# tomneda/DABstar

Measured on NVIDIA B200. Metric: Mode I DAB frames/s decoded (IQ->Viterbi), higher is better.
Workload: dtype f32

## Files before the change

dabstar_b200/csrc/ofdm_kernels.cu:

```cuda
#include "fft2048.cuh"
#include "kernels.h"
#include "devcache.h"

#include <algorithm>
#include <cstdlib>
#include <type_traits>

namespace dab
{
namespace
{
template <int FMT> struct Raw;
template <> struct Raw<FMT_U8> { typedef unsigned short type; typedef unsigned reg; };
template <> struct Raw<FMT_I16> { typedef short2 type; typedef short2 reg; };
template <> struct Raw<FMT_CF32> { typedef float2 type; typedef float2 reg; };

__device__ __forceinline__ float2 to_cf(unsigned v)
{
  const float2 m = make_float2(__uint_as_float(__byte_perm(v, 0x4B000000u, 0x7540)), __uint_as_float(__byte_perm(v, 0x4B000000u, 0x7541)));
  const float2 f = __fadd2_rn(m, make_float2(-8388608.0f, -8388608.0f));
  return __ffma2_rn(f, make_float2(1.0f / 128.0f, 1.0f / 128.0f), make_float2(-127.38f / 128.0f, -127.38f / 128.0f));
}
__device__ __forceinline__ float2 to_cf(short2 v) { return __fmul2_rn(make_float2((float)v.x, (float)v.y), make_float2(1.0f / 32768.0f, 1.0f / 32768.0f)); }
__device__ __forceinline__ float2 to_cf(float2 v) { return v; }
// ... 645 lines not shown
  fft2048_to_smem(v, tw, smem, tid);
  for (int i = tid; i < T_U; i += FFT_THREADS) ref_arg_conj[i] = smem[fft_nat(i)];
}

struct CpInt
{
  int p1, p2, s1, s2;
};
__device__ __forceinline__ unsigned dp4a_uu(unsigned a, unsigned b, unsigned c)
{
  unsigned d;
  asm("dp4a.u32.u32 %0, %1, %2, %3;" : "=r"(d) : "r"(a), "r"(b), "r"(c));
  return d;
}
__device__ __forceinline__ int dp4a_us(unsigned a, unsigned b_signed, int c)
{
  int d;
  asm("dp4a.u32.s32 %0, %1, %2, %3;" : "=r"(d) : "r"(a), "r"(b_signed), "r"(c));
  return d;
}
__device__ __forceinline__ void cp_int_add(CpInt & t, unsigned aw, unsigned bw)
{
  t.p1 = (int)dp4a_uu(aw, bw, (unsigned)t.p1);
  const unsigned bs = __byte_perm(bw, 0u, 0x2301);
  t.p2 = (int)dp4a_uu(aw & 0xff00ff00u, bs, (unsigned)t.p2);
  t.p2 -= (int)dp4a_uu(aw & 0x00ff00ffu, bs, 0u);
  t.s1 = (int)dp4a_uu(aw, 0x01010101u, dp4a_uu(bw, 0x01010101u, (unsigned)t.s1));
  t.s2 = dp4a_us(aw, 0x01ff01ffu, dp4a_us(bw, 0xff01ff01u, t.s2));
}
__device__ __forceinline__ int warp_sum_int(int v)
{
#pragma unroll
  for (int o = 16; o > 0; o >>= 1) v += __shfl_xor_sync(0xffffffffu, v, o);
  return v;
}
__device__ __forceinline__ float2 cp_int_finish(const CpInt * red, int n_syms)
{
  long long p1 = 0, p2 = 0, s1 = 0, s2 = 0;
  for (int w = 0; w < 8; w++) { p1 += red[w].p1; p2 += red[w].p2; s1 += red[w].s1; s2 += red[w].s2; }
  const double c = 127.38, n = (double)n_syms * (double)T_G;
  return make_float2((float)(((double)p1 - c * (double)s1 + 2.0 * n * c * c) * (1.0 / 16384.0)), (float)(((double)p2 - c * (double)s2) * (1.0 / 16384.0)));
}

template <int FMT>
__global__ void __launch_bounds__(256) k_cp_corr(const FrameDesc * __restrict__ frames, int n_frames, const RecInput * __restrict__ recs, float2 * __restrict__ cp)
{
  __shared__ float2 red[8];
  __shared__ CpInt redi[8];
  for (int fi = blockIdx.x; fi < n_frames; fi += gridDim.x)
  {
    const FrameDesc fd = frames[fi];
    const RecInput rin = recs[fd.rec];
    const long long base = fd.sym0 + T_U;
    float2 acc = make_float2(0.0f, 0.0f);
    CpInt ti = { 0, 0, 0, 0 };
    typedef typename Raw<FMT>::type T;
    const int lane = threadIdx.x & 31;
    for (int sym = threadIdx.x >> 5; sym < fd.n_syms; sym += 8)
    {
      const T * pp = reinterpret_cast<const T *>(rin.iq) + base + (long long)sym * T_S + lane;
      typename Raw<FMT>::reg ra[16], rb[16];
#pragma unroll
      for (int k = 0; k < 16; k++)
      {
        if (lane + 32 * k < T_G) { ra[k] = pp[32 * k + T_U]; rb[k] = pp[32 * k]; }
        else { ra[k] = typename Raw<FMT>::reg(); rb[k] = typename Raw<FMT>::reg(); }
      }
#pragma unroll
      for (int k = 0; k < 16; k++)
      {
        if (lane + 32 * k < T_G)
        {
          if constexpr (FMT == FMT_U8) cp_int_add(ti, ra[k], rb[k]);
          else
          {
            const float2 a = to_cf(ra[k]), b = to_cf(rb[k]);
            acc.x += a.x * b.x + a.y * b.y;
            acc.y += a.y * b.x - a.x * b.y;
          }
        }
      }
    }
    if constexpr (FMT == FMT_U8)
    {
      ti.p1 = warp_sum_int(ti.p1); ti.p2 = warp_sum_int(ti.p2); ti.s1 = warp_sum_int(ti.s1); ti.s2 = warp_sum_int(ti.s2);
      if ((threadIdx.x & 31) == 0) redi[threadIdx.x >> 5] = ti;
      __syncthreads();
      if (threadIdx.x == 0) cp[fi] = cp_int_finish(redi, fd.n_syms);
    }
    else
    {
      acc.x = warp_sum(acc.x);
      acc.y = warp_sum(acc.y);
      if ((threadIdx.x & 31) == 0) red[threadIdx.x >> 5] = acc;
      __syncthreads();
      if (threadIdx.x == 0)
      {
        float2 s = red[0];
        for (int w = 1; w < 8; w++) { s.x += red[w].x; s.y += red[w].y; }
        cp[fi] = s;
      }
    }
    __syncthreads();
  }
}

constexpr int CPB_STAGES = 4;
constexpr int CPB_COPY = 1024;
constexpr int CPB_SMEM = 8 * CPB_STAGES * 2 * CPB_COPY;

__global__ void __launch_bounds__(256) k_cp_corr_bulk(const FrameDesc * __restrict__ frames, int n_frames, const RecInput * __restrict__ recs, float2 * __restrict__ cp)
{
  extern __shared__ __align__(128) unsigned char cpb_ring[];
  __shared__ unsigned long long cpb_bar[8 * CPB_STAGES];
  __shared__ CpInt red[8];
  const int lane = threadIdx.x & 31, warp = threadIdx.x >> 5;
  unsigned char * ring = cpb_ring + warp * (CPB_STAGES * 2 * CPB_COPY);
  const unsigned ring_s = smem_addr_u32(ring), bar_s = smem_addr_u32(cpb_bar + warp * CPB_STAGES);
  if (lane == 0)
  {
#pragma unroll
    for (int b = 0; b < CPB_STAGES; b++) mbar_init(bar_s + 8u * (unsigned)b, 1);
    asm volatile("fence.mbarrier_init.release.cluster;" ::: "memory");
    asm volatile("fence.proxy.async.shared::cta;" ::: "memory");
  }
  __syncthreads();

  struct Cursor
  {
    int fi, sym, n_syms;
    long long base, n;
    const unsigned char * iq;
  };
  auto enter = [&](Cursor & c) {
    while (c.fi < n_frames)
    {
      const FrameDesc & fd = frames[c.fi];
      c.n_syms = fd.n_syms;
      if (warp < c.n_syms)
      {
        const RecInput rin = recs[fd.rec];
        c.base = fd.sym0 + T_U;
        c.n = rin.n;
        c.iq = static_cast<const unsigned char *>(rin.iq);
        c.sym = warp;
        return;
      }
      c.fi += (int)gridDim.x;
    }
  };
  auto advance = [&](Cursor & c) {
    c.sym += 8;
    if (c.sym >= c.n_syms) { c.fi += (int)gridDim.x; enter(c); }
  };
  auto first_sample = [](const Cursor & c) { return c.base + (long long)c.sym * T_S; };
  auto by_copy = [&](const Cursor & c) { const long long s0 = first_sample(c); return s0 >= 8 && s0 + T_U + T_G + 8 <= c.n; };
  auto issue = [&](const Cursor & c, int b) {
    if (c.fi < n_frames && by_copy(c) && lane == 0)
    {
      const unsigned long long a = (unsigned long long)(c.iq + 2 * first_sample(c)) & ~15ull;
      const unsigned dst = ring_s + (unsigned)(b * 2 * CPB_COPY), bar = bar_s + 8u * (unsigned)b;
      mbar_expect_tx(bar, 2u * CPB_COPY);
      bulk_g2s(dst, reinterpret_cast<const void *>(a), CPB_COPY, bar);
      bulk_g2s(dst + CPB_COPY, reinterpret_cast<const void *>(a + 2ull * T_U), CPB_COPY, bar);
    }
  };

  Cursor ahead;
  ahead.fi = (int)blockIdx.x;
  ahead.sym = 0; ahead.n_syms = 0; ahead.base = 0; ahead.n = 0; ahead.iq = nullptr;
  enter(ahead);
  Cursor cur = ahead;
#pragma unroll 1
  for (int b = 0; b < CPB_STAGES && ahead.fi < n_frames; b++) { issue(ahead, b); advance(ahead); }
  int stage = 0;
  unsigned phase_bits = 0;

  for (int fi = blockIdx.x; fi < n_frames; fi += gridDim.x)
  {
    CpInt ti = { 0, 0, 0, 0 };
    const int n_syms = frames[fi].n_syms;
    while (cur.fi == fi)
    {
      if (by_copy(cur))
      {
        mbar_wait(bar_s + 8u * (unsigned)stage, (phase_bits >> stage) & 1u);
        phase_bits ^= 1u << stage;
        const int off = (int)((unsigned long long)(cur.iq + 2 * first_sample(cur)) & 15ull);
        const uint4 * sp = reinterpret_cast<const uint4 *>(ring + stage * 2 * CPB_COPY) + lane;
        uint4 va[2], vb[2];
#pragma unroll
        for (int it = 0; it < 2; it++) { vb[it] = sp[32 * it]; va[it] = sp[32 * it + CPB_COPY / 16]; }
        if (lane == 0)
        {
          unsigned * w = reinterpret_cast<unsigned *>(&va[0]);
          unsigned * u = reinterpret_cast<unsigned *>(&vb[0]);
#pragma unroll
          for (int j = 0; j < 4; j++)
          {
            const int drop = min(max(off - 4 * j, 0), 4);
            const unsigned m = drop >= 4 ? 0u : 0xffffffffu << (8 * drop);
            w[j] &= m;
            u[j] &= m;
          }
        }
        if (lane == 31)
        {
          unsigned * w = reinterpret_cast<unsigned *>(&va[1]);
          unsigned * u = reinterpret_cast<unsigned *>(&vb[1]);
#pragma unroll
          for (int j = 0; j < 4; j++)
          {
            const int keep = min(max(off - 4 * j, 0), 4);
            const unsigned m = keep >= 4 ? 0xffffffffu : ~(0xffffffffu << (8 * keep));
            w[j] &= m;
            u[j] &= m;
          }
        }
#pragma unroll
        for (int it = 0; it < 2; it++)
        {
          cp_int_add(ti, va[it].x, vb[it].x);
          cp_int_add(ti, va[it].y, vb[it].y);
          cp_int_add(ti, va[it].z, vb[it].z);
          cp_int_add(ti, va[it].w, vb[it].w);
        }
      }
      else
      {
        const unsigned short * pp = reinterpret_cast<const unsigned short *>(cur.iq) + first_sample(cur) + lane;
        unsigned ra[16], rb[16];
#pragma unroll
        for (int k = 0; k < 16; k++)
        {
          if (lane + 32 * k < T_G) { ra[k] = pp[32 * k + T_U]; rb[k] = pp[32 * k]; }
          else { ra[k] = 0; rb[k] = 0; }
        }
#pragma unroll
        for (int k = 0; k < 16; k++) cp_int_add(ti, ra[k], rb[k]);
      }
      __syncwarp();
      asm volatile("fence.proxy.async.shared::cta;" ::: "memory");
      issue(ahead, stage);
      if (ahead.fi < n_frames) advance(ahead);
      advance(cur);
      stage = stage + 1 == CPB_STAGES ? 0 : stage + 1;
    }
    ti.p1 = warp_sum_int(ti.p1); ti.p2 = warp_sum_int(ti.p2); ti.s1 = warp_sum_int(ti.s1); ti.s2 = warp_sum_int(ti.s2);
    if (lane == 0) red[warp] = ti;
    __syncthreads();
    if (threadIdx.x == 0) cp[fi] = cp_int_finish(red, n_syms);
    __syncthreads();
  }
}

constexpr int DM3_RING = 64;
constexpr int DM3_ROW4 = K_CARR / 2;

__device__ __forceinline__ float rcp_ftz(float a) { float r; asm("rcp.approx.ftz.f32 %0, %1;" : "=f"(r) : "f"(a)); return r; }
__device__ __forceinline__ float rsqrt_ftz(float a) { float r; asm("rsqrt.approx.ftz.f32 %0, %1;" : "=f"(r) : "f"(a)); return r; }
__device__ __forceinline__ float sqrt_ftz(float a) { float r; asm("sqrt.approx.ftz.f32 %0, %1;" : "=f"(r) : "f"(a)); return r; }

__device__ __forceinline__ unsigned long long ld_volatile_global_b64(const unsigned long long * p)
{
  unsigned long long v;
  asm volatile("ld.relaxed.gpu.global.b64 %0, [%1];" : "=l"(v) : "l"(p) : "memory");
  return v;
}
__device__ __forceinline__ void st_volatile_global_b64(unsigned long long * p, unsigned long long v)
{
  asm volatile("st.relaxed.gpu.global.b64 [%0], %1;" ::"l"(p), "l"(v) : "memory");
}

__device__ __forceinline__ float2 f2(float a) { return make_float2(a, a); }
__device__ __forceinline__ float2 neg2(float2 a) { return make_float2(-a.x, -a.y); }
__device__ __forceinline__ float2 add2(float2 a, float2 b) { return __fadd2_rn(a, b); }
__device__ __forceinline__ float2 mul2(float2 a, float2 b) { return __fmul2_rn(a, b); }
__device__ __forceinline__ float2 fma2(float2 a, float2 b, float2 c) { return __ffma2_rn(a, b, c); }

struct CarrierPair
{
  float2 integ, stddev, mean_pow, mean_sigma, null_pow;
};

__device__ __forceinline__ float2 folded_phase2(float2 re, float2 im)
{
  const float ax0 = fabsf(re.x), ay0 = fabsf(im.x), ax1 = fabsf(re.y), ay1 = fabsf(im.y);
  const float2 mn = make_float2(fminf(ax0, ay0), fminf(ax1, ay1));
  const float2 t = mul2(mn, make_float2(rcp_ftz(fmaxf(ax0, ay0)), rcp_ftz(fmaxf(ax1, ay1))));
  const float2 z = mul2(t, t);
  float2 p = f2(0.00681177107617259f);
  p = fma2(p, z, f2(-0.033604156225919724f));
  p = fma2(p, z, f2(0.07962360233068466f));
  p = fma2(p, z, f2(-0.13233338296413422f));
  p = fma2(p, z, f2(0.19807815551757812f));
  p = fma2(p, z, f2(-0.3331736922264099f));
  p = fma2(p, z, f2(0.9999961256980896f));
  const float2 a = mul2(p, t);
  const bool m0 = (ay0 > ax0) != ((__float_as_int(re.x) ^ __float_as_int(im.x)) < 0);
  const bool m1 = (ay1 > ax1) != ((__float_as_int(re.y) ^ __float_as_int(im.y)) < 0);
  return make_float2(m0 ? PI_2_F - a.x : a.x, m1 ? PI_2_F - a.y : a.y);
}

template <int SOFT>
__device__ __forceinline__ void dm4_pair(CarrierPair & st, float2 xr, float2 xi, float2 rr, float2 ri, float2 ref_abs, float2 ref_inv, float2 cterm,
                                         float2 & o_re, float2 & o_im, float2 & r_abs, float2 & pow_acc)
{
  constexpr float ALPHA = 0.005f;
  const float2 re = mul2(fma2(xi, ri, mul2(xr, rr)), ref_inv);
  const float2 im = mul2(fma2(neg2(xr), ri, mul2(xi, rr)), ref_inv);
  const float2 t = add2(cterm, st.integ), a2 = mul2(t, t);
  const float2 rx = fma2(a2, fma2(a2, f2(3.679168224334716796875e-2f), f2(-0.495580852031707763671875f)), f2(0.9994032382965087890625f));
  const float2 ry = mul2(neg2(t), fma2(a2, f2(-0.16034401953220367431640625f), f2(0.99903142452239990234375f)));
  const float2 zr = fma2(neg2(im), ry, mul2(re, rx));
  const float2 zi = fma2(im, rx, mul2(re, ry));
  const float2 dv = add2(folded_phase2(zr, zi), f2(-PI_4_F));
  const float2 in = fma2(dv, f2(0.2f * ALPHA), st.integ);
  st.integ = make_float2(fminf(fmaxf(in.x, -20.0f * RAD_PER_DEG_F), 20.0f * RAD_PER_DEG_F), fminf(fmaxf(in.y, -20.0f * RAD_PER_DEG_F), 20.0f * RAD_PER_DEG_F));
  st.stddev = fma2(fma2(dv, dv, neg2(st.stddev)), f2(ALPHA), st.stddev);
  const float2 pw = fma2(zr, zr, mul2(zi, zi));
  st.mean_pow = fma2(add2(pw, neg2(st.mean_pow)), f2(ALPHA), st.mean_pow);
  pow_acc = fma2(pow_acc, f2(POW_ALL_DECAY), pw);
  const float2 lvl = make_float2(sqrt_ftz(st.mean_pow.x), sqrt_ftz(st.mean_pow.y));
  const float2 dr = fma2(lvl, f2(-0.70710678118654752440f), make_float2(fabsf(zr.x), fabsf(zr.y)));
  const float2 di = fma2(lvl, f2(-0.70710678118654752440f), make_float2(fabsf(zi.x), fabsf(zi.y)));
  st.mean_sigma = fma2(add2(fma2(dr, dr, mul2(di, di)), neg2(st.mean_sigma)), f2(ALPHA), st.mean_sigma);
  float2 sig = add2(st.mean_pow, neg2(st.null_pow));
  if (sig.x <= 0.0f) sig.x = 0.1f;
  if (sig.y <= 0.0f) sig.y = 0.1f;
  const float2 inv_z = make_float2(rsqrt_ftz(pw.x), rsqrt_ftz(pw.y));
  float2 w1;
  if (SOFT == 2) w1 = ref_abs;
  else
  {
    const float2 den = mul2(fma2(sig, f2(0.7f), st.null_pow), st.mean_sigma);
    const float2 g = mul2(sig, make_float2(rcp_ftz(den.x), rcp_ftz(den.y)));
    if (SOFT == 1) w1 = mul2(ref_abs, g);
    else
    {
      const float2 q = mul2(ref_abs, inv_z);
      w1 = mul2(mul2(make_float2(sqrt_ftz(q.x), sqrt_ftz(q.y)), lvl), g);
    }
  }
  r_abs = mul2(mul2(pw, inv_z), w1);
  o_re = mul2(zr, w1);
  o_im = mul2(zi, w1);
}

__device__ __forceinline__ void dm4_fix_saturated(int & a, int & b, int & c, int & e)
{
  a = a == 0x7fffffff ? 0 : a; b = b == 0x7fffffff ? 0 : b; c = c == 0x7fffffff ? 0 : c; e = e == 0x7fffffff ? 0 : e;
}

constexpr int DM5_T = 128;
constexpr int DM5_SLICES = K_CARR / 4 / DM5_T;
constexpr int DM5_WARPS = K_CARR / 128;
constexpr int DM5_PF = 8;

__device__ __forceinline__ float dm5_total(const unsigned long long * slot, unsigned long long w, unsigned tag, int lane)
{
  while (__any_sync(0xffffffffu, lane < DM5_WARPS && (unsigned)(w >> 32) != tag)) w = ld_volatile_global_b64(slot + (lane < DM5_WARPS ? lane : 0));
  float v = lane < DM5_WARPS ? __uint_as_float((unsigned)w) : 0.0f;
#pragma unroll
  for (int o = 16; o > 0; o >>= 1) v += __shfl_xor_sync(0xffffffffu, v, o);
  return v;
}

template <int SOFT, int LAG, bool QUAL>
__global__ void __launch_bounds__(DM5_T, 4) k_demap5(const DemapWork * __restrict__ work, const FrameDesc * __restrict__ frames,
                                                      const uint8_t * __restrict__ null_is_tii, const float2 * __restrict__ X,
                                                      const int16_t * __restrict__ rel_of_k, OfdmStateDev * __restrict__ states,
                                                      int16_t * __restrict__ soft, unsigned long long * __restrict__ ring, unsigned * __restrict__ ticket,
                                                      FrameQualSnap * __restrict__ qsnap)
{
  constexpr int STASH = LAG + 1;
  constexpr int T = DM5_T;
  static_assert((STASH & (STASH - 1)) == 0, "stash depth must be a power of two");
  static_assert(DM3_RING > 2 * LAG + 2, "a ring slot must not be overwritten while a slower warp may still read it");
  extern __shared__ float4 dm5_smem[];
  __shared__ unsigned s_ticket;
  if (threadIdx.x == 0) s_ticket = atomicAdd(ticket, 1u);
  __syncthreads();
  float4 * stash = dm5_smem;
  float4 * rowbuf = dm5_smem + STASH * T * 2;
  int * orow_ring = reinterpret_cast<int *>(rowbuf + DM5_PF * T * 2) + (threadIdx.x >> 5);
  const int w = (int)s_ticket / DM5_SLICES, slice = (int)s_ticket - w * DM5_SLICES;
  const DemapWork wk = work[w];
  const int tid = threadIdx.x, lane = tid & 31;
  const int t_rec = slice * T + tid;
  const int gw = t_rec >> 5;
  const int k0 = 4 * t_rec;
  unsigned long long * my_ring = ring + (size_t)w * DM3_RING * DM5_WARPS;

  const OfdmStateDev & sd = states[wk.state_in];
  CarrierPair sa, sb;
  float2 pow_a = f2(0.f), pow_b = f2(0.f);
  if (wk.reset) sa = sb = CarrierPair{ f2(0.f), f2(0.f), f2(0.f), f2(0.f), f2(0.f) };
  else
  {
    const float4 v0 = *reinterpret_cast<const float4 *>(sd.integ + k0), v1 = *reinterpret_cast<const float4 *>(sd.stddev + k0),
                 v2 = *reinterpret_cast<const float4 *>(sd.mean_pow + k0), v3 = *reinterpret_cast<const float4 *>(sd.mean_sigma + k0),
                 v4 = *reinterpret_cast<const float4 *>(sd.null_pow + k0), v5 = *reinterpret_cast<const float4 *>(sd.pow_acc + k0);
    sa = CarrierPair{ make_float2(v0.x, v0.y), make_float2(v1.x, v1.y), make_float2(v2.x, v2.y), make_float2(v3.x, v3.y), make_float2(v4.x, v4.y) };
    sb = CarrierPair{ make_float2(v0.z, v0.w), make_float2(v1.z, v1.w), make_float2(v2.z, v2.w), make_float2(v3.z, v3.w), make_float2(v4.z, v4.w) };
    pow_a = make_float2(v5.x, v5.y);
    pow_b = make_float2(v5.z, v5.w);
  }
  const float mean_value0 = sd.mean_value;
  const float pow_carry0 = wk.reset ? 1.0f : sd.pow_carry;
  const float2 gka = make_float2((float)(K_CARR / 2 - rel_of_k[k0]) / (float)(K_CARR / 2), (float)(K_CARR / 2 - rel_of_k[k0 + 1]) / (float)(K_CARR / 2));
  const float2 gkb = make_float2((float)(K_CARR / 2 - rel_of_k[k0 + 2]) / (float)(K_CARR / 2), (float)(K_CARR / 2 - rel_of_k[k0 + 3]) / (float)(K_CARR / 2));
  constexpr float W2 = SOFT == 0 ? -100.0f : -140.0f;

  const int total_rows = wk.n_frames * X_ROWS;
  const float4 * rows = reinterpret_cast<const float4 *>(X + (size_t)(total_rows > 0 ? frames[wk.desc_first].xslot : 0) * X_ROWS * K_CARR) + 2 * t_rec;
  const unsigned rowbuf_addr = smem_addr_u32(rowbuf + 2 * tid);
#pragma unroll
  for (int i = 0; i < DM5_PF; i++)
  {
    if (i < total_rows)
    {
      cp_async16(rowbuf_addr + (unsigned)(i * T) * 32u, rows + (size_t)i * DM3_ROW4);
      cp_async16(rowbuf_addr + (unsigned)(i * T) * 32u + 16u, rows + (size_t)i * DM3_ROW4 + 1);
    }
    cp_async_commit();
  }

  float2 rra = f2(0.f), ria = f2(0.f), ref_abs_a = f2(0.f), ref_inv_a = f2(0.f);
  float2 rrb = f2(0.f), rib = f2(0.f), ref_abs_b = f2(0.f), ref_inv_b = f2(0.f);
  int g = 0;
  int q = 0;
  unsigned long long pre = 0;

  auto emit = [&](int d, int o_row, float total) {
    if (o_row < 0) return;
    const float w2 = d == 0 ? rcp_ftz(mean_value0) * W2 : rcp_ftz(total) * (W2 * (float)K_CARR);
    const float4 ra = stash[((d & (STASH - 1)) * T + tid) * 2], rb = stash[((d & (STASH - 1)) * T + tid) * 2 + 1];
    const float2 are = mul2(make_float2(ra.x, ra.y), f2(w2)), aim = mul2(make_float2(ra.z, ra.w), f2(w2));
    const float2 bre = mul2(make_float2(rb.x, rb.y), f2(w2)), bim = mul2(make_float2(rb.z, rb.w), f2(w2));
    int a0 = __float2int_rz(are.x), a1 = __float2int_rz(are.y), a2 = __float2int_rz(aim.x), a3 = __float2int_rz(aim.y);
    int b0 = __float2int_rz(bre.x), b1 = __float2int_rz(bre.y), b2 = __float2int_rz(bim.x), b3 = __float2int_rz(bim.y);
    if (max(max(max(a0, a1), max(a2, a3)), max(max(b0, b1), max(b2, b3))) == 0x7fffffff) { dm4_fix_saturated(a0, a1, a2, a3); dm4_fix_saturated(b0, b1, b2, b3); }
    int16_t * o = soft + (size_t)o_row * SYM_BITS;
    reinterpret_cast<uint2 *>(o)[t_rec] = make_uint2(__byte_perm((unsigned)a0, (unsigned)a1, 0x5410), __byte_perm((unsigned)b0, (unsigned)b1, 0x5410));
    reinterpret_cast<uint2 *>(o + K_CARR)[t_rec] = make_uint2(__byte_perm((unsigned)a2, (unsigned)a3, 0x5410), __byte_perm((unsigned)b2, (unsigned)b3, 0x5410));
  };
  auto wsum = [](float v) {
#pragma unroll
    for (int o = 16; o > 0; o >>= 1) v += __shfl_xor_sync(0xffffffffu, v, o);
    return v;
  };
  float4 cur_a, cur_b;
  auto next_row = [&]() {
    cp_async_wait<DM5_PF - 1>();
    const unsigned slot = (unsigned)((q & (DM5_PF - 1)) * T);
    cur_a = rowbuf[(slot + tid) * 2];
    cur_b = rowbuf[(slot + tid) * 2 + 1];
    if (q + DM5_PF < total_rows)
    {
      cp_async16(rowbuf_addr + slot * 32u, rows + (size_t)(q + DM5_PF) * DM3_ROW4);
      cp_async16(rowbuf_addr + slot * 32u + 16u, rows + (size_t)(q + DM5_PF) * DM3_ROW4 + 1);
    }
    cp_async_commit();
    q++;
  };
  auto set_reference = [&]() {
    rra = make_float2(cur_a.x, cur_a.y); ria = make_float2(cur_a.z, cur_a.w);
    rrb = make_float2(cur_b.x, cur_b.y); rib = make_float2(cur_b.z, cur_b.w);
    const float2 pa = fma2(rra, rra, mul2(ria, ria)), pb = fma2(rrb, rrb, mul2(rib, rib));
    ref_inv_a = make_float2(rsqrt_ftz(pa.x), rsqrt_ftz(pa.y));
    ref_inv_b = make_float2(rsqrt_ftz(pb.x), rsqrt_ftz(pb.y));
    ref_abs_a = mul2(pa, ref_inv_a);
    ref_abs_b = mul2(pb, ref_inv_b);
  };
  float part_prev = 0.0f;
  const bool upper = (lane & 16) != 0;
  int q_wait_g = -1, q_wait = 0;
  auto q_mean_value = [&](int d, float total) {
    if (QUAL && d == q_wait_g)
    {
      if (t_rec == 0) qsnap[q_wait].mean_value = total / (float)K_CARR;
      q_wait_g = -1;
    }
  };

  for (int fi = 0; fi < wk.n_frames; fi++)
  {
    const FrameDesc fd = frames[wk.desc_first + fi];
    const float cfac = fd.clock_err / 1024.0f * PI_F;
    const float2 cterm_a = mul2(f2(cfac), gka), cterm_b = mul2(f2(cfac), gkb);
    const int n_syms = fd.n_syms;
    const int out_row0 = fi < wk.warmup ? -(1 << 30) : fd.slot * 75;
    const bool tii = null_is_tii != nullptr && null_is_tii[wk.desc_first + fi];
    next_row();
    set_reference();
    for (int sym = 1; sym <= 75; sym++)
    {
      next_row();
      if (sym > n_syms) continue;
      const int d = g - LAG;
      const float b_in = lane < DM5_WARPS ? __uint_as_float((unsigned)pre) : 0.0f;
      const bool tags_ok = __all_sync(0xffffffffu, lane >= DM5_WARPS || (unsigned)(pre >> 32) == (unsigned)d);
      const unsigned long long pre_used = pre;
      if (d >= 0 && lane < DM5_WARPS) pre = ld_volatile_global_b64(my_ring + (size_t)(d & (DM3_RING - 1)) * DM5_WARPS + lane);
      float v = (upper ? b_in : part_prev) + __shfl_xor_sync(0xffffffffu, upper ? part_prev : b_in, 16);
#pragma unroll
      for (int o = 8; o > 0; o >>= 1) v += __shfl_xor_sync(0xffffffffu, v, o);
      const float tot_fast = __shfl_sync(0xffffffffu, v, 16);
      float2 a_re, a_im, a_abs, b_re, b_im, b_abs;
      dm4_pair<SOFT>(sa, make_float2(cur_a.x, cur_a.y), make_float2(cur_a.z, cur_a.w), rra, ria, ref_abs_a, ref_inv_a, cterm_a, a_re, a_im, a_abs, pow_a);
      dm4_pair<SOFT>(sb, make_float2(cur_b.x, cur_b.y), make_float2(cur_b.z, cur_b.w), rrb, rib, ref_abs_b, ref_inv_b, cterm_b, b_re, b_im, b_abs, pow_b);
      part_prev = (a_abs.x + a_abs.y) + (b_abs.x + b_abs.y);
      stash[((g & (STASH - 1)) * T + tid) * 2] = make_float4(a_re.x, a_re.y, a_im.x, a_im.y);
      stash[((g & (STASH - 1)) * T + tid) * 2 + 1] = make_float4(b_re.x, b_re.y, b_im.x, b_im.y);
      if (lane == 0) orow_ring[(g & (STASH - 1)) * (T >> 5)] = out_row0 + (sym - 1);
      __syncwarp();
      if (lane == 0 && g > 0)
        st_volatile_global_b64(my_ring + (size_t)((g - 1) & (DM3_RING - 1)) * DM5_WARPS + gw,
                               ((unsigned long long)(unsigned)g << 32) | (unsigned long long)__float_as_uint(v));
      if (d >= 0)
      {
        float tot = tot_fast;
        if (d > 0 && !tags_ok) tot = dm5_total(my_ring + (size_t)((d - 1) & (DM3_RING - 1)) * DM5_WARPS, pre_used, (unsigned)d, lane);
        emit(d, orow_ring[(d & (STASH - 1)) * (T >> 5)], tot);
        q_mean_value(d, tot);
      }
      g++;
      set_reference();
    }
    next_row();
    if (n_syms == 75 && !tii)
    {
      constexpr float MIN_POW = (1.0f / 32767.0f) * (1.0f / 32767.0f);
      const float2 xra = make_float2(cur_a.x, cur_a.y), xia = make_float2(cur_a.z, cur_a.w), xrb = make_float2(cur_b.x, cur_b.y), xib = make_float2(cur_b.z, cur_b.w);
      const float2 pa = add2(fma2(xra, xra, mul2(xia, xia)), f2(MIN_POW)), pb = add2(fma2(xrb, xrb, mul2(xib, xib)), f2(MIN_POW));
      sa.null_pow = fma2(add2(pa, neg2(sa.null_pow)), f2(0.05f), sa.null_pow);
      sb.null_pow = fma2(add2(pb, neg2(sb.null_pow)), f2(0.05f), sb.null_pow);
    }
    if (QUAL && out_row0 >= 0 && n_syms == 75)
    {
      FrameQualSnap & qs = qsnap[wk.desc_first + fi];
      *reinterpret_cast<float4 *>(qs.stddev + k0) = make_float4(sa.stddev.x, sa.stddev.y, sb.stddev.x, sb.stddev.y);
      *reinterpret_cast<float4 *>(qs.null_pow + k0) = make_float4(sa.null_pow.x, sa.null_pow.y, sb.null_pow.x, sb.null_pow.y);
      *reinterpret_cast<float4 *>(qs.pow_acc + k0) = make_float4(pow_a.x, pow_a.y, pow_b.x, pow_b.y);
      if (t_rec == 0) qs.pow_carry = pow_carry0 * powf(POW_ALL_DECAY, (float)g);
      q_wait_g = g;
      q_wait = wk.desc_first + fi;
    }
  }
  cp_async_wait<0>();
  if (g > 0)
  {
    const float part = wsum(part_prev);
    if (lane == 0)
      st_volatile_global_b64(my_ring + (size_t)((g - 1) & (DM3_RING - 1)) * DM5_WARPS + gw,
                             ((unsigned long long)(unsigned)g << 32) | (unsigned long long)__float_as_uint(part));
  }
#pragma unroll
  for (int i = LAG - 1; i >= 0; i--)
  {
    const int d = g - 1 - i;
    if (d < 0) continue;
    float tot = 0.0f;
    if (d >= 1)
    {
      const unsigned long long * slot = my_ring + (size_t)((d - 1) & (DM3_RING - 1)) * DM5_WARPS;
      unsigned long long word = 0;
      if (lane < DM5_WARPS) word = ld_volatile_global_b64(slot + lane);
      tot = dm5_total(slot, word, (unsigned)d, lane);
    }
    emit(d, orow_ring[(d & (STASH - 1)) * (T >> 5)], tot);
    q_mean_value(d, tot);
  }
  if (!QUAL && wk.state_out < 0) return;
  float tot_last = mean_value0 * (float)K_CARR;
  if (gw == 0 && g > 0)
  {
    unsigned long long word = 0;
    const unsigned long long * slot = my_ring + (size_t)((g - 1) & (DM3_RING - 1)) * DM5_WARPS;
    if (lane < DM5_WARPS) word = ld_volatile_global_b64(slot + lane);
    tot_last = dm5_total(slot, word, (unsigned)g, lane);
  }
  if (QUAL)
  {
    q_mean_value(g, tot_last);
    if (wk.state_out < 0) return;
  }
  OfdmStateDev & so = states[wk.state_out];
  *reinterpret_cast<float4 *>(so.integ + k0) = make_float4(sa.integ.x, sa.integ.y, sb.integ.x, sb.integ.y);
  *reinterpret_cast<float4 *>(so.stddev + k0) = make_float4(sa.stddev.x, sa.stddev.y, sb.stddev.x, sb.stddev.y);
  *reinterpret_cast<float4 *>(so.mean_pow + k0) = make_float4(sa.mean_pow.x, sa.mean_pow.y, sb.mean_pow.x, sb.mean_pow.y);
  *reinterpret_cast<float4 *>(so.mean_sigma + k0) = make_float4(sa.mean_sigma.x, sa.mean_sigma.y, sb.mean_sigma.x, sb.mean_sigma.y);
  *reinterpret_cast<float4 *>(so.null_pow + k0) = make_float4(sa.null_pow.x, sa.null_pow.y, sb.null_pow.x, sb.null_pow.y);
  *reinterpret_cast<float4 *>(so.pow_acc + k0) = make_float4(pow_a.x, pow_a.y, pow_b.x, pow_b.y);
  if (gw == 0 && lane == 0) so.mean_value = g > 0 ? tot_last / (float)K_CARR : mean_value0;
  if (t_rec == 0) so.pow_carry = pow_carry0 * powf(POW_ALL_DECAY, (float)g);
}

constexpr int DIP_THREADS = 256;
constexpr int DIP_BLOCK = 1024;
constexpr float LEVEL_ALPHA = 0.00001f;

template <int FMT> __device__ __forceinline__ float sample_abs(const void * iq, long long i)
{
  const float2 v = load_sample<FMT>(iq, i);
  return sqrtf(v.x * v.x + v.y * v.y);
}
template <int FMT> __device__ __forceinline__ typename Raw<FMT>::reg sample_raw(const void * iq, long long i)
{
  return (typename Raw<FMT>::reg)reinterpret_cast<const typename Raw<FMT>::type *>(iq)[i];
}
template <int FMT> __device__ __forceinline__ float raw_abs(typename Raw<FMT>::reg r)
{
  const float2 v = to_cf(r);
  return sqrtf(v.x * v.x + v.y * v.y);
}

template <int FMT>
__global__ void __launch_bounds__(DIP_THREADS) k_dip_search(const DipWork * __restrict__ work, const RecInput * __restrict__ recs, DipResult * __restrict__ out)
{
  __shared__ float mag[DIP_BLOCK + 64];
  __shared__ float lvl[DIP_BLOCK];
  __shared__ float2 scan_ab[DIP_THREADS];
  __shared__ float redf[DIP_THREADS / 32];
  __shared__ int found;
  const DipWork wk = work[blockIdx.x];
  const RecInput rin = recs[wk.rec];
  const int tid = threadIdx.x;
  const long long p0 = wk.pos;
  const float loga = log1pf(-LEVEL_ALPHA);

  const long long hist = p0 < (1LL << 21) ? p0 : (1LL << 21);
  float acc = 0.0f;
  {
    float ru[8];
#pragma unroll
    for (int u = 0; u < 8; u++) ru[u] = expf((float)(DIP_THREADS * u) * loga);
    long long i = tid;
    for (; i + 7LL * DIP_THREADS < hist; i += 8LL * DIP_THREADS)
    {
      typename Raw<FMT>::reg rw[8];
#pragma unroll
      for (int u = 0; u < 8; u++) rw[u] = sample_raw<FMT>(rin.iq, p0 - 1 - (i + (long long)u * DIP_THREADS));
      float m[8];
#pragma unroll
      for (int u = 0; u < 8; u++) m[u] = raw_abs<FMT>(rw[u]);
      const float w = expf((float)i * loga);
#pragma unroll
      for (int u = 0; u < 8; u++) acc = fmaf(m[u], w * ru[u], acc);
    }
    for (; i < hist; i += DIP_THREADS) acc = fmaf(sample_abs<FMT>(rin.iq, p0 - 1 - i), expf((float)i * loga), acc);
  }
  acc = warp_sum(acc);
  if ((tid & 31) == 0) redf[tid >> 5] = acc;
  __syncthreads();
  float s_level = 0.0f;
  for (int w = 0; w < DIP_THREADS / 32; w++) s_level += redf[w];
  s_level = LEVEL_ALPHA * s_level + (hist == p0 ? 0.1f * expf((float)(p0 + wk.abs0) * loga) : 0.0f);
  __syncthreads();

  int phase = 0;
  long long dip_i = -1;
  int status = -1;
  long long end_pos = p0;
  const float a1 = 1.0f - LEVEL_ALPHA;
  typename Raw<FMT>::reg nx[DIP_BLOCK / DIP_THREADS];
  auto fetch = [&](long long b0) {
    const bool inside = p0 + b0 + DIP_BLOCK <= rin.n;
#pragma unroll
    for (int u = 0; u < DIP_BLOCK / DIP_THREADS; u++) nx[u] = inside ? sample_raw<FMT>(rin.iq, p0 + b0 + tid + u * DIP_THREADS) : typename Raw<FMT>::reg();
  };
  fetch(0);
  if (tid < 49) mag[tid] = 0.0f;
  for (long long b0 = 0; status < 0; b0 += DIP_BLOCK)
  {
    if (p0 + b0 + DIP_BLOCK > rin.n) { status = 3; end_pos = rin.n; break; }
    if (b0 > 0)
    {
      float keep = 0.0f;
      if (tid < 49) keep = mag[DIP_BLOCK + tid];
      __syncthreads();
      if (tid < 49) mag[tid] = keep;
    }
#pragma unroll
    for (int u = 0; u < DIP_BLOCK / DIP_THREADS; u++) mag[49 + tid + u * DIP_THREADS] = raw_abs<FMT>(nx[u]);
    __syncthreads();
    fetch(b0 + DIP_BLOCK);
    float A = 1.0f, B = 0.0f;
#pragma unroll
    for (int q = 0; q < 4; q++) { const float m = mag[49 + 4 * tid + q]; B = a1 * B + LEVEL_ALPHA * m; A *= a1; }
    {
      const int lane = tid & 31, wp = tid >> 5;
#pragma unroll
      for (int o = 1; o < 32; o <<= 1)
      {
        const float pa = __shfl_up_sync(0xffffffffu, A, o), pb = __shfl_up_sync(0xffffffffu, B, o);
        if (lane >= o) { B = fmaf(A, pb, B); A *= pa; }
      }
      if (lane == 31) scan_ab[wp] = make_float2(A, B);
      __syncthreads();
      float s = s_level;
      for (int w = 0; w < wp; w++) { const float2 ab = scan_ab[w]; s = fmaf(ab.x, s, ab.y); }
      const float ea = __shfl_up_sync(0xffffffffu, A, 1), eb = __shfl_up_sync(0xffffffffu, B, 1);
      if (lane > 0) s = fmaf(ea, s, eb);
#pragma unroll
      for (int q = 0; q < 4; q++) { s = a1 * s + LEVEL_ALPHA * mag[49 + 4 * tid + q]; lvl[4 * tid + q] = s; }
      if (tid == DIP_THREADS - 1) scan_ab[DIP_THREADS / 32].x = s;
    }
    if (tid == 0) found = 0x7fffffff;
    __syncthreads();
    const float s_after = scan_ab[DIP_THREADS / 32].x;
    int from = 0;
    while (true)
    {
      int best = 0x7fffffff;
      {
        float c0 = 0.0f, c1 = 0.0f;
#pragma unroll 5
        for (int j = 0; j < 50; j += 2) { c0 += mag[4 * tid + j]; c1 += mag[4 * tid + j + 1]; }
        float c = c0 + c1;
#pragma unroll
        for (int q = 0; q < 4; q++)
        {
          const int i = 4 * tid + q;
          const long long gi = b0 + i;
          if (q > 0) c += mag[i + 49] - mag[i - 1];
          if (i < from || (phase == 0 && gi < 49) || best != 0x7fffffff) continue;
          const float mean = c / 50.0f;
          const bool hit = phase == 0 ? !(mean > 0.55f * lvl[i]) : !(mean < 0.75f * lvl[i]);
          if (hit) best = i;
        }
      }
      if (best != 0x7fffffff) atomicMin(&found, best);
      __syncthreads();
      const int f = found;
      __syncthreads();
      if (tid == 0) found = 0x7fffffff;
      __syncthreads();
      if (phase == 0)
      {
        const long long lim = 49 + (long long)T_F;
        const long long gi = f == 0x7fffffff ? (long long)1 << 60 : b0 + f;
        if (gi <= lim) { phase = 1; dip_i = gi; from = f; continue; }
        if (b0 + DIP_BLOCK - 1 >= lim + 1) { status = 1; end_pos = p0 + lim + 2; }
        break;
      }
      else
      {
        const long long lim = dip_i + T_N + 70;
        const long long gi = f == 0x7fffffff ? (long long)1 << 60 : b0 + f;
        if (gi <= lim) { status = 0; end_pos = p0 + gi + 1; }
        else if (b0 + DIP_BLOCK - 1 >= lim + 1) { status = 2; end_pos = p0 + lim + 2; }
        break;
      }
    }
    s_level = s_after;
    __syncthreads();
  }
  if (tid == 0)
  {
    if (end_pos > rin.n) { end_pos = rin.n; status = 3; }
    out[blockIdx.x].pos = end_pos;
    out[blockIdx.x].status = status;
    out[blockIdx.x].s_level = s_level;
  }
}

__device__ __forceinline__ float ingest_value(const unsigned char * p, int container, int msb_first, float inv_scaler, const float * __restrict__ lut)
{
  switch (container)
  {
  case 0: case 1: case 6: return lut[p[0]];
  case 7:
  {
    const unsigned v = ((unsigned)p[3] << 24) | (p[2] << 16) | (p[1] << 8) | p[0];
    return (float)(int)v * 4.656612873077393e-10f;
  }
  case 2:
  {
    const int v = msb_first ? ((p[0] << 8) | p[1]) : ((p[1] << 8) | p[0]);
    return (float)(short)v * inv_scaler;
  }
  case 3:
  {
    int v = msb_first ? ((p[0] << 16) | (p[1] << 8) | p[2]) : ((p[2] << 16) | (p[1] << 8) | p[0]);
    if (v & 0x800000) v |= (int)0xFF000000;
    return (float)v * inv_scaler;
  }
  case 4:
  {
    const unsigned v = msb_first ? (((unsigned)p[0] << 24) | (p[1] << 16) | (p[2] << 8) | p[3]) : (((unsigned)p[3] << 24) | (p[2] << 16) | (p[1] << 8) | p[0]);
    return (float)(int)v * inv_scaler;
  }
  default:
  {
    const unsigned v = msb_first ? (((unsigned)p[0] << 24) | (p[1] << 16) | (p[2] << 8) | p[3]) : (((unsigned)p[3] << 24) | (p[2] << 16) | (p[1] << 8) | p[0]);
    return __uint_as_float(v);
  }
  }
}

__global__ void __launch_bounds__(256) k_ingest_convert(const unsigned char * __restrict__ src, int container, int msb_first, int iq_order, float inv_scaler,
                                                        const float * __restrict__ lut, long long n, float2 * __restrict__ dst)
{
  const int bytes = (container <= 1 || container == 6) ? 1 : (container == 2 ? 2 : (container == 3 ? 3 : 4));
  for (long long i = (long long)blockIdx.x * blockDim.x + threadIdx.x; i < n; i += (long long)gridDim.x * blockDim.x)
  {
    float2 o;
    if (iq_order <= 1)
    {
      const float a = ingest_value(src + (2 * i) * bytes, container, msb_first, inv_scaler, lut);
      const float b = ingest_value(src + (2 * i + 1) * bytes, container, msb_first, inv_scaler, lut);
      o = iq_order == 0 ? make_float2(a, b) : make_float2(b, a);
    }
    else
    {
      const float a = ingest_value(src + i * bytes, container, msb_first, inv_scaler, lut);
      o = iq_order == 2 ? make_float2(a, 0.0f) : make_float2(0.0f, a);
    }
    dst[i] = o;
  }
}

__global__ void __launch_bounds__(256) k_resample_linear(const float2 * __restrict__ in, long long n_in, int block_in, int shift,
                                                         const short * __restrict__ base, const float * __restrict__ frac,
                                                         long long n_out, float2 * __restrict__ out)
{
  for (long long o = (long long)blockIdx.x * blockDim.x + threadIdx.x; o < n_out; o += (long long)gridDim.x * blockDim.x)
  {
    const long long b = o >> 11;
    const int j = (int)(o & 2047);
    const long long lo = b * block_in + base[j] - shift;
// ... 214 lines not shown
```

Baseline: 805,900.

## Software-pipeline demap: split carrier pair into front/back stages across symbols

Splits the per-symbol demap into a front stage (derotation, phase tracking) and a back stage (power and soft-weight statistics). The front of the next symbol now runs right after the back of the current one, so independent arithmetic can overlap the cross-warp ring reduction. Launch bounds are also lowered per LAG to leave room for the extra live registers. The price is more register pressure and fewer resident CTAs per SM for the larger lags.

Result: faster. 819,400, median of 6 (+1.7%).

```diff
diff --git a/dabstar_b200/csrc/ofdm_kernels.cu b/dabstar_b200/csrc/ofdm_kernels.cu
--- a/dabstar_b200/csrc/ofdm_kernels.cu
+++ b/dabstar_b200/csrc/ofdm_kernels.cu
@@ -971,9 +971,8 @@
   return make_float2(m0 ? PI_2_F - a.x : a.x, m1 ? PI_2_F - a.y : a.y);
 }
 
-template <int SOFT>
-__device__ __forceinline__ void dm4_pair(CarrierPair & st, float2 xr, float2 xi, float2 rr, float2 ri, float2 ref_abs, float2 ref_inv, float2 cterm,
-                                         float2 & o_re, float2 & o_im, float2 & r_abs, float2 & pow_acc)
+__device__ __forceinline__ void dm4_front(CarrierPair & st, float2 xr, float2 xi, float2 rr, float2 ri, float2 ref_inv, float2 cterm,
+                                          float2 & zr, float2 & zi)
 {
   constexpr float ALPHA = 0.005f;
   const float2 re = mul2(fma2(xi, ri, mul2(xr, rr)), ref_inv);
@@ -981,12 +980,19 @@
   const float2 t = add2(cterm, st.integ), a2 = mul2(t, t);
   const float2 rx = fma2(a2, fma2(a2, f2(3.679168224334716796875e-2f), f2(-0.495580852031707763671875f)), f2(0.9994032382965087890625f));
   const float2 ry = mul2(neg2(t), fma2(a2, f2(-0.16034401953220367431640625f), f2(0.99903142452239990234375f)));
-  const float2 zr = fma2(neg2(im), ry, mul2(re, rx));
-  const float2 zi = fma2(im, rx, mul2(re, ry));
+  zr = fma2(neg2(im), ry, mul2(re, rx));
+  zi = fma2(im, rx, mul2(re, ry));
   const float2 dv = add2(folded_phase2(zr, zi), f2(-PI_4_F));
   const float2 in = fma2(dv, f2(0.2f * ALPHA), st.integ);
   st.integ = make_float2(fminf(fmaxf(in.x, -20.0f * RAD_PER_DEG_F), 20.0f * RAD_PER_DEG_F), fminf(fmaxf(in.y, -20.0f * RAD_PER_DEG_F), 20.0f * RAD_PER_DEG_F));
   st.stddev = fma2(fma2(dv, dv, neg2(st.stddev)), f2(ALPHA), st.stddev);
+}
+
+template <int SOFT>
+__device__ __forceinline__ void dm4_back(CarrierPair & st, float2 zr, float2 zi, float2 ref_abs, float2 & o_re, float2 & o_im, float2 & r_abs,
+                                         float2 & pow_acc)
+{
+  constexpr float ALPHA = 0.005f;
   const float2 pw = fma2(zr, zr, mul2(zi, zi));
   st.mean_pow = fma2(add2(pw, neg2(st.mean_pow)), f2(ALPHA), st.mean_pow);
   pow_acc = fma2(pow_acc, f2(POW_ALL_DECAY), pw);
@@ -1025,6 +1031,7 @@
 constexpr int DM5_SLICES = K_CARR / 4 / DM5_T;
 constexpr int DM5_WARPS = K_CARR / 128;
 constexpr int DM5_PF = 8;
+constexpr int dm5_ctas_per_sm(int lag) { return lag == 15 ? 2 : (lag == 7 ? 3 : 4); }
 
 __device__ __forceinline__ float dm5_total(const unsigned long long * slot, unsigned long long w, unsigned tag, int lane)
 {
@@ -1036,7 +1043,7 @@
 }
 
 template <int SOFT, int LAG, bool QUAL>
-__global__ void __launch_bounds__(DM5_T, 4) k_demap5(const DemapWork * __restrict__ work, const FrameDesc * __restrict__ frames,
+__global__ void __launch_bounds__(DM5_T, dm5_ctas_per_sm(LAG)) k_demap5(const DemapWork * __restrict__ work, const FrameDesc * __restrict__ frames,
                                                       const uint8_t * __restrict__ null_is_tii, const float2 * __restrict__ X,
                                                       const int16_t * __restrict__ rel_of_k, OfdmStateDev * __restrict__ states,
                                                       int16_t * __restrict__ soft, unsigned long long * __restrict__ ring, unsigned * __restrict__ ticket,
@@ -1097,6 +1104,7 @@
 
   float2 rra = f2(0.f), ria = f2(0.f), ref_abs_a = f2(0.f), ref_inv_a = f2(0.f);
   float2 rrb = f2(0.f), rib = f2(0.f), ref_abs_b = f2(0.f), ref_inv_b = f2(0.f);
+  float2 za_r = f2(0.f), za_i = f2(0.f), zref_abs_a = f2(0.f), zb_r = f2(0.f), zb_i = f2(0.f), zref_abs_b = f2(0.f);
   int g = 0;
   int q = 0;
   unsigned long long pre = 0;
@@ -1161,12 +1169,14 @@
     const int n_syms = fd.n_syms;
     const int out_row0 = fi < wk.warmup ? -(1 << 30) : fd.slot * 75;
     const bool tii = null_is_tii != nullptr && null_is_tii[wk.desc_first + fi];
-    next_row();
-    set_reference();
-    for (int sym = 1; sym <= 75; sym++)
-    {
-      next_row();
-      if (sym > n_syms) continue;
+    auto front = [&]() {
+      dm4_front(sa, make_float2(cur_a.x, cur_a.y), make_float2(cur_a.z, cur_a.w), rra, ria, ref_inv_a, cterm_a, za_r, za_i);
+      dm4_front(sb, make_float2(cur_b.x, cur_b.y), make_float2(cur_b.z, cur_b.w), rrb, rib, ref_inv_b, cterm_b, zb_r, zb_i);
+      zref_abs_a = ref_abs_a;
+      zref_abs_b = ref_abs_b;
+      set_reference();
+    };
+    auto symbol = [&](int sym, bool more) {
       const int d = g - LAG;
       const float b_in = lane < DM5_WARPS ? __uint_as_float((unsigned)pre) : 0.0f;
       const bool tags_ok = __all_sync(0xffffffffu, lane >= DM5_WARPS || (unsigned)(pre >> 32) == (unsigned)d);
@@ -1177,8 +1187,9 @@
       for (int o = 8; o > 0; o >>= 1) v += __shfl_xor_sync(0xffffffffu, v, o);
       const float tot_fast = __shfl_sync(0xffffffffu, v, 16);
       float2 a_re, a_im, a_abs, b_re, b_im, b_abs;
-      dm4_pair<SOFT>(sa, make_float2(cur_a.x, cur_a.y), make_float2(cur_a.z, cur_a.w), rra, ria, ref_abs_a, ref_inv_a, cterm_a, a_re, a_im, a_abs, pow_a);
-      dm4_pair<SOFT>(sb, make_float2(cur_b.x, cur_b.y), make_float2(cur_b.z, cur_b.w), rrb, rib, ref_abs_b, ref_inv_b, cterm_b, b_re, b_im, b_abs, pow_b);
+      dm4_back<SOFT>(sa, za_r, za_i, zref_abs_a, a_re, a_im, a_abs, pow_a);
+      dm4_back<SOFT>(sb, zb_r, zb_i, zref_abs_b, b_re, b_im, b_abs, pow_b);
+      if (more) front();
       part_prev = (a_abs.x + a_abs.y) + (b_abs.x + b_abs.y);
       stash[((g & (STASH - 1)) * T + tid) * 2] = make_float4(a_re.x, a_re.y, a_im.x, a_im.y);
       stash[((g & (STASH - 1)) * T + tid) * 2 + 1] = make_float4(b_re.x, b_re.y, b_im.x, b_im.y);
@@ -1195,8 +1206,22 @@
         q_mean_value(d, tot);
       }
       g++;
-      set_reference();
-    }
+    };
+    next_row();
+    set_reference();
+    const int n = max(min(n_syms, 75), 0);
+    if (n > 0)
+    {
+      next_row();
+      front();
+    }
+    for (int sym = 1; sym < n; sym++)
+    {
+      next_row();
+      symbol(sym, true);
+    }
+    if (n > 0) symbol(n, false);
+    for (int sym = n + 1; sym <= 75; sym++) next_row();
     next_row();
     if (n_syms == 75 && !tii)
     {
```
